# alinjar1996/manipulator_mujoco

Hardware: AMD Instinct MI355X
Metric: candidate rollouts/sec (N×H steps) UR5e scene, 1/2/4/8 MI355X (higher is better)
Workload: dtype f32; 1 GPU; C3 scene_mjx: UR5e+Hand-E arm + object.xml box (URD/scene_mjx.xml), Newton(1 it, 5 ls), 4096 candidates x 50 steps per GPU, order-10 Bernstein, dt 0.05; candidates_per_gpu=4096, horizon=50, global_batch=4096, parallelism=dp1 (candidate shards; key exchange), world_size_seen=1, backend=single process, gpus_visible=1, launcher=single process, exchange=none (one rank: the fused atomic-min key is the global best)

## Files before the change

### manipulator_mujoco_amd/csrc/dev_model.h

```cpp
#pragma once
#include <algorithm>
#include <atomic>
#include <cfloat>
#include <cmath>
#include <cstdarg>
#include <cstdio>
#include <cstring>
#include <limits>
#include <string>
#include <thread>
#include <vector>

#include "../../include/mpcr.h"
#include "model_frames.h"
#include "rollout.h"

namespace mpcr {

struct DevOptions {
  int newton_reuse = 1;
  int m_slab = 0;
  int w2_lead_max = W2_LEAD_MAX;
  uint64_t start_scramble = 0;
};
// ... 314 lines not shown
  }
  {
    int ts[DX_NTREE], te[DX_NTREE];
    bool ok = true;
    for (int t = 0; t < DX_NTREE; t++) ts[t] = te[t] = -1;
    for (int i = 0; i < m.nv && ok; i++) {
      const int b = d.dof_body[i], t = b >= 0 ? d.body_tree[b] : -1;
      if (t < 0 || t >= DX_NTREE) { ok = false; break; }
      if (ts[t] < 0) ts[t] = i;
      else if (te[t] != i) ok = false;
      te[t] = i + 1;
    }
    for (int i = 0; i < m.nv && ok; i++) {
      const int t = d.body_tree[d.dof_body[i]];
      d.mc_c0[i] = std::min(ts[t] & ~3, SmemW::NVW - SmemW::MCW);
      if (te[t] - d.mc_c0[i] > SmemW::MCW) ok = false;
    }
    d.mc_n = ok && m.nv * SmemW::MCW <= SmemW::MC ? m.nv : 0;
    if (opt.m_slab) d.mc_n = 0;
    d.w2_lead_max = std::max(-1, std::min(W2_LEAD_MAX, opt.w2_lead_max));
  }
  for (int i = 0; i < m.nq; i++) d.qpos_init[i] = (float)m.qpos_init[i];
  for (int i = 0; i < m.nv; i++) d.qvel_init[i] = (float)m.qvel_init[i];
  std::vector<int> gmap(m.ngeom, -1);
  int ng = 0;
  for (int p = 0; p < m.npair; p++)
    for (int g : {m.pair_geom1[p], m.pair_geom2[p]})
      if (gmap[g] < 0) gmap[g] = ng++;
  if (ng > DX_NG || ng > WAVE) return dev_fail(err, MPCR_EMODEL, "%d collision geoms > %d", ng, DX_NG < WAVE ? DX_NG : WAVE);
  d.ngeom = ng;
  for (int g = 0; g < m.ngeom; g++) {
    int i = gmap[g];
    if (i < 0) continue;
    int b = m.geom_bodyid[g];
    d.geom_type[i] = m.geom_type[g];
    d.geom_rbound[i] = (float)m.geom_rbound[g];
    d.geom_hulladr[i] = m.geom_hulladr[g];
    d.geom_hullnum[i] = m.geom_hullnum[g];
    d.geom_lutadr[i] = lutadr[g];
    d.geom_faceadr[i] = m.geom_faceadr[g];
    d.geom_facenum[i] = m.geom_faceadr[g] >= 0 ? m.geom_facenum[g] : 0;
    d.geom_cornadr[i] = m.geom_cornadr[g];
    for (int k = 0; k < 3; k++) d.geom_size[i][k] = (float)m.geom_size[g][k];
    if (dmap[b] >= 0) {
      d.geom_body[i] = dmap[b];
      for (int k = 0; k < 3; k++) d.geom_pos[i][k] = (float)m.geom_pos[g][k];
      for (int k = 0; k < 4; k++) d.geom_quat[i][k] = (float)m.geom_quat[g][k];
    } else {
      d.geom_body[i] = -1;
      double r[3], q[4];
      step_detail::rot(r, f.wquat[b], m.geom_pos[g]);
// ... 254 lines not shown
```

### manipulator_mujoco_amd/csrc/engine.hip

```cpp
#include <hip/hip_runtime.h>
#include <dlfcn.h>

#include <algorithm>
#include <atomic>
#include <cmath>
#include <cstdarg>
#include <cstdio>
#include <cstring>
#include <string>
#include <vector>

#include "../../include/mpcr.h"
#include "mpcr_device.h"

#include "rollout.h"
#include "dev_model.h"
#include "step_table.h"

#ifndef MPCR_SEG_STEPS_DEFAULT
#define MPCR_SEG_STEPS_DEFAULT 7
#endif
#ifndef MPCR_SEG_GROUPS_DEFAULT
#define MPCR_SEG_GROUPS_DEFAULT 2
#endif
// ... 289 lines not shown
  HIPCHK(hipSetDevice(device));
  hipDeviceProp_t prop;
  HIPCHK(hipGetDeviceProperties(&prop, device));
  if (std::strncmp(prop.gcnArchName, "gfx950", 6) != 0)
    return fail(MPCR_ENODEV, "device %d is %s; libmpcr is built for gfx950 only", device, prop.gcnArchName);
  auto* e = new mpcr_engine;
  auto refuse = [e](int rc) { mpcr_engine_free(e); return rc; };
  e->device = device;
  e->max_n = max_n;
  e->H = horizon;
  e->nbasis = nbasis;
  e->host = m->m;
  const mpcr_model_t& h = e->host;
  DevOptions opt;
  opt.newton_reuse = env_int_or("MPCR_NEWTON_REUSE", 1);
  opt.m_slab = env_int_or("MPCR_M_SLAB", 0);
  opt.w2_lead_max = env_int_or("MPCR_W2_LEAD_MAX", W2_LEAD_MAX);
  opt.start_scramble = g_start_scramble.load();
  DevTables t;
  std::string err;
  if (int rc = compile_dev_model(h, opt, e->dev, t, err)) return refuse(fail(rc, "%s", err.c_str()));
  e->wide = needs_wide(h, e->dev);
  std::vector<StepTable> step;
  if (!e->wide) {
    step.resize(1);
    if (build_step_table(h, step[0]) != 0) return refuse(fail(MPCR_EMODEL, "model exceeds the step table's capacities"));
  }
  DevBufs& mem = e->mem;
  if (h.nhullv > 0) {
    e->dev.hull_vert = as_gmem(mem.upload(t.hull_vert));
    e->dev.hull_info = as_gmem(mem.upload(t.hull_info));
    e->dev.hull_adjv = as_gmem(mem.upload(t.hull_adjv));
    e->dev.hull_head = as_gmem(mem.upload(t.hull_head));
    e->dev.hull_lut = as_gmem(mem.upload(t.hull_lut));
  }
  if (h.nface > 0) {
    e->dev.face_plane = as_gmem(mem.upload(t.face_plane));
    e->dev.face_vinfo = as_gmem(mem.upload(t.face_vinfo));
    e->dev.face_vert = as_gmem(mem.alloc<int>(h.nfacev, h.face_vert, h.nfacev));
    e->dev.vert_finfo = as_gmem(mem.upload(t.vert_finfo));
    e->dev.vert_face = as_gmem(mem.alloc<int>(h.nvface, h.vert_face, h.nvface));
    e->dev.cone_cell = as_gmem(mem.upload(t.cone_cell));
    e->dev.cone_face = as_gmem(mem.upload(t.cone_face));
  }
  static_assert(sizeof(DevModel) % alignof(mpcr::StepTable) == 0, "the step table's alignment behind the device model");
  const int nc = h.nctrl;
  const size_t rows = (size_t)max_n + 1;
  const size_t nhints = 2 * (size_t)max_n * (e->wide ? SmemW::NHINT : 1);
  e->d_model = reinterpret_cast<DevModel*>(mem.alloc<char>(sizeof(DevModel) + sizeof(StepTable),
                                                           reinterpret_cast<const char*>(&e->dev), sizeof(DevModel)));
  if (e->d_model && !e->wide &&
      hipMemcpy(e->d_model + 1, step.data(), sizeof(StepTable), hipMemcpyHostToDevice) != hipSuccess)
    mem.rc = MPCR_EHIP;
  e->d_pdot = mem.alloc<float>((size_t)horizon * nbasis, pdot, (size_t)horizon * nbasis);
  e->d_in = mem.alloc<float>((size_t)max_n * nc * (horizon > nbasis ? horizon : nbasis));
  e->d_cost = mem.alloc<float>((size_t)max_n * 4);
  e->d_theta = mem.alloc<float>((size_t)max_n * nc * horizon);
  e->d_thetadot = mem.alloc<float>((size_t)max_n * nc * horizon);
  e->d_key = mem.alloc<unsigned long long>(1);
  e->d_status = mem.alloc<int>(max_n);
  e->d_idx = mem.alloc<int>(max_n);
  e->d_slot_prev = mem.alloc<float>(rows * (h.nslot > 0 ? h.nslot : 1));
  e->d_jx = mem.alloc<float>(rows * (e->wide ? (SmemW::MAXEFC - SmemW::JL + 1) * SmemW::LDJ
                                             : (SmemN::MAXEFC - SmemN::JL + 1) * SmemN::LDJ));
  e->d_hints = mem.alloc<short>(nhints);
  e->d_pace = mem.alloc<unsigned>(MPCR_PACE_SLOTS);
  e->d_mslab = mem.alloc<float>(rows * (e->wide ? SmemW::NVW * SmemW::LD : 1));
  e->d_td = mem.alloc<float>(rows * (size_t)(nc > 0 ? nc : 1) * (size_t)horizon);
  if (!mem.rc && (hipMemset(e->d_hints, 0xff, sizeof(short) * nhints) != hipSuccess ||
                  hipMemset(e->d_pace, 0xff, sizeof(unsigned) * MPCR_PACE_SLOTS) != hipSuccess))
    mem.rc = MPCR_EHIP;
  if (e->wide) {
    e->seg_steps = env_int_or("MPCR_SEG_STEPS", MPCR_SEG_STEPS_DEFAULT);
    e->seg_groups = std::max(1, std::min(MPCR_SEG_MAXG, env_int_or("MPCR_SEG_GROUPS", MPCR_SEG_GROUPS_DEFAULT)));
    if (e->seg_steps > 0 && e->seg_steps < horizon) {
// ... 834 lines not shown
```

### manipulator_mujoco_amd/csrc/model_frames.h

```cpp
#pragma once
#include <math.h>
#include <stdint.h>
#include <string.h>

#include "../../include/mpcr_model.h"

namespace mpcr {

enum { ST_BK_FREE = 1, ST_BK_HINGE = 2, ST_BK_SLIDE = 3, ST_BK_WELD = 4 };

namespace step_detail {
inline void qmul(double r[4], const double a[4], const double b[4]) {
  const double t[4] = {a[0] * b[0] - a[1] * b[1] - a[2] * b[2] - a[3] * b[3],
                       a[0] * b[1] + a[1] * b[0] + a[2] * b[3] - a[3] * b[2],
                       a[0] * b[2] - a[1] * b[3] + a[2] * b[0] + a[3] * b[1],
                       a[0] * b[3] + a[1] * b[2] - a[2] * b[1] + a[3] * b[0]};
  memcpy(r, t, sizeof(t));
}
inline void q2m(double m[9], const double q[4]) {
  const double w = q[0], x = q[1], y = q[2], z = q[3];
  m[0] = 1 - 2 * (y * y + z * z); m[1] = 2 * (x * y - w * z); m[2] = 2 * (x * z + w * y);
  m[3] = 2 * (x * y + w * z); m[4] = 1 - 2 * (x * x + z * z); m[5] = 2 * (y * z - w * x);
  m[6] = 2 * (x * z - w * y); m[7] = 2 * (y * z + w * x); m[8] = 1 - 2 * (x * x + y * y);
}
// ... 51 lines not shown
      f.anc[i] = -1;
    } else {
      memcpy(f.bpos[i], m.body_pos[b], sizeof(f.bpos[i]));
      memcpy(f.bquat[i], m.body_quat[b], sizeof(f.bquat[i]));
      f.anc[i] = f.dmap[p];
    }
    if (f.kind[i] == ST_BK_FREE) f.anc[i] = -1;
    f.depth[i] = f.anc[i] < 0 ? 1 : f.depth[f.anc[i]] + 1;
    f.maxdepth = f.depth[i] > f.maxdepth ? f.depth[i] : f.maxdepth;
    int t = -1;
    for (int k = 0; k < f.ntree; k++)
      if (roots[k] == m.body_rootid[b]) t = k;
    if (t < 0) { roots[f.ntree] = m.body_rootid[b]; t = f.ntree++; }
    f.tree[i] = t;
  }
  for (int i = 0; i < m.nv; i++) {
    const int j = m.dof_jntid[i], sub = i - m.jnt_dofadr[j];
    f.dof_kind[i] = m.jnt_type[j] == MPCR_JNT_HINGE ? 0 : (m.jnt_type[j] == MPCR_JNT_SLIDE ? 1 : (sub < 3 ? 2 : 3));
    f.dof_sub[i] = sub < 3 ? sub : sub - 3;
  }
  return 0;
}

inline float pair_margin_f(const mpcr_model_t& m, int p) { return (float)(m.pair_margin[p] - m.pair_gap[p]); }
inline bool pair_frictionless(const mpcr_model_t& m, int p) { return m.pair_condim[p] == 1; }
inline bool jnt_limit_row(const mpcr_model_t& m, int j) {
  return m.jnt_limited[j] && (m.jnt_type[j] == MPCR_JNT_SLIDE || m.jnt_type[j] == MPCR_JNT_HINGE);
}
inline float jnt_range_f(const mpcr_model_t& m, int j, int k) { return (float)m.jnt_range[j][k]; }
inline float jnt_margin_f(const mpcr_model_t& m, int j) { return (float)m.jnt_margin[j]; }
inline float dof_invweight_f(const mpcr_model_t& m, int i) { return (float)m.dof_invweight0[i]; }
inline float eq_diag_f(const mpcr_model_t& m, int e) {
  double diag = 0;
  if (m.eq_type[e] == MPCR_EQ_JOINT) {
    diag = m.dof_invweight0[m.jnt_dofadr[m.eq_obj1[e]]];
    if (m.eq_obj2[e] >= 0) diag += m.dof_invweight0[m.jnt_dofadr[m.eq_obj2[e]]];
  } else if (m.eq_type[e] == MPCR_EQ_CONNECT) {
    diag = m.body_invweight0[m.eq_obj1[e]][0] + m.body_invweight0[m.eq_obj2[e]][0];
  }
  return (float)diag;
}

}
```

### manipulator_mujoco_amd/csrc/rollout.hip

```cpp
#pragma once
#include "rollout.h"
#include "step_table.h"
#include "../../include/mpcr_model.h"

namespace mpcr {

#ifdef MPCR_PROFILE
#define PROF_DECL unsigned long long prof_acc[32] = {0}; unsigned long long prof_last = __builtin_amdgcn_s_memtime();
#define STAMP(i)                                              \
  do {                                                        \
    unsigned long long now_ = __builtin_amdgcn_s_memtime();   \
    prof_acc[i] += now_ - prof_last;                          \
    prof_last = now_;                                         \
  } while (0)
#define PROF_FLUSH                                                          \
  if (lane == 0 && args.prof)                                               \
    for (int i_ = 0; i_ < 32; i_++) atomicAdd(&args.prof[i_ + 32 * (threadIdx.x >> 6)], prof_acc[i_]);
#ifdef MPCR_PROFILE_COUNTS
#define PROF_COUNT(m, i)                                                                  \
  do {                                                                                    \
    if ((m)->prof && (int)__lane_id() == __builtin_ctzll(__ballot(1))) atomicAdd((m)->prof + (i), 1ull); \
  } while (0)
#else
#define PROF_COUNT(m, i)
// ... 11 lines not shown
#define PROF_DECL
#define STAMP(i)
#define PROF_FLUSH
#define PROF_COUNT(m, i)
#endif
#define PACE_SETPRIO() \
  if (pace) {   \
  const int ahead = __popcll(__ballot(lane < 16 && lane != pace_own && pace_v != ~0u && pace_v > (unsigned)t)); \
  if (ahead >= 3) __builtin_amdgcn_s_setprio(3); \
  else if (ahead == 2) __builtin_amdgcn_s_setprio(2); \
  else if (ahead == 1) __builtin_amdgcn_s_setprio(1); \
  else __builtin_amdgcn_s_setprio(0); \
  }

#ifndef MPCR_CB_SKIP
#define MPCR_CB_SKIP 1
#endif
#ifdef MPCR_STOP_AFTER
#define STOP_AT(k) \
  if (MPCR_STOP_AFTER == (k)) continue;
#else
#define STOP_AT(k)
#endif


#if defined(__HIP_DEVICE_COMPILE__)
#define ASSUME_GLOBAL(p) __builtin_assume(!__builtin_amdgcn_is_shared((const void*)(p)) && \
                                          !__builtin_amdgcn_is_private((const void*)(p)))
#define ASSUME_LDS(p) __builtin_assume(__builtin_amdgcn_is_shared((const void*)(p)))
#define ASSUME_PRIVATE(p) __builtin_assume(__builtin_amdgcn_is_private((const void*)(p)))
#else
#define ASSUME_GLOBAL(p)
#define ASSUME_LDS(p)
#define ASSUME_PRIVATE(p)
#endif
__device__ __forceinline__ const MPCR_GMEM DevModel* uniform_model(const DevModel* p) {
  const unsigned long long a = reinterpret_cast<unsigned long long>(p);
  const unsigned lo = __builtin_amdgcn_readfirstlane((unsigned)a), hi = __builtin_amdgcn_readfirstlane((unsigned)(a >> 32));
  return reinterpret_cast<const MPCR_GMEM DevModel*>(((unsigned long long)hi << 32) | lo);
}

#ifndef MPCR_STEP_TABLE
#define MPCR_STEP_TABLE 7
#endif
template <class S> constexpr bool kStepKin = !S::WIDE && (MPCR_STEP_TABLE & 1) != 0;
template <class S> constexpr bool kStepDof = !S::WIDE && (MPCR_STEP_TABLE & 2) != 0;
template <class S> constexpr bool kStepRow = !S::WIDE && (MPCR_STEP_TABLE & 4) != 0;
__device__ __forceinline__ const StepTable* step_table(const DevModel* m) {
  return reinterpret_cast<const StepTable*>(m + 1);
}
template <class R>
__device__ __forceinline__ float4 recq(const R& r, int q) {
  return reinterpret_cast<const float4*>(&r)[q];
}

__device__ __forceinline__ float rdlane(float v, int l) {
  return __int_as_float(__builtin_amdgcn_readlane(__float_as_int(v), l));
}
template <int CTRL>
__device__ __forceinline__ float dppf(float v) {
  return __int_as_float(__builtin_amdgcn_update_dpp(0, __float_as_int(v), CTRL, 0xF, 0xF, false));
}
template <int CTRL, int ROWS>
__device__ __forceinline__ float dppf_rows(float v) {
  return __int_as_float(__builtin_amdgcn_update_dpp(0, __float_as_int(v), CTRL, ROWS, 0xF, false));
}
__device__ __forceinline__ float wsum_ref(float v) {
  v += dppf<0xB1>(v);
  v += dppf<0x4E>(v);
  v += dppf<0x124>(v);
  v += dppf<0x128>(v);
  v += dppf_rows<0x142, 0xA>(v);
// ... 1303 lines not shown
    idx[0] = ia; idx[1] = ib; idx[2] = ic; idx[3] = beats(bap, bbp) ? iap : ibp;
  }
#pragma unroll
  for (int j = 0; j < 4; j++) {
    bool dup = idx[j] < 0;
#pragma unroll
    for (int t = 0; t < j; t++) dup |= idx[t] == idx[j];
    const int L = idx[j] < 0 ? 0 : idx[j];
    const float Pj[3] = {__shfl(P[0], L), __shfl(P[1], L), __shfl(P[2], L)};
    const float dj = __shfl(dk, L);
    if (lane == q) {
      dist[j] = dup ? 1e30f : dj;
#pragma unroll
      for (int e = 0; e < 3; e++) { pos[j][e] = Pj[e] - 0.5f * dj * nr[e] + c[e]; nrm[j][e] = sg * nr[e]; }
    }
  }
  if (lane == q) nsl = 4;
  PSTAMP(m, 28);
}

template <class S>
__device__ __forceinline__ int narrow_lane(const DevModel* __restrict__ m, const S& s, short* hints, int p, float dist[4],
                            float pos[4][3], float nrm[4][3], float* dbg = nullptr) {
  const int g1 = m->pair_g1[p], g2 = m->pair_g2[p];
  const int func = m->pair_func[p];
  const float* x1 = s.gxpos[g1];
  const float* x2 = s.gxpos[g2];
  const float* R1 = s.gxmat[g1];
  const float* R2 = s.gxmat[g2];
  const float* s1 = m->geom_size[g1];
  const float* s2 = m->geom_size[g2];
#pragma unroll
  for (int k = 0; k < 4; k++) dist[k] = 1e30f;
  if (func == 0) {
    float n[3] = {R1[2], R1[5], R1[8]}, ax[3] = {R2[2], R2[5], R2[8]};
    float r = s2[0], hl = s2[1];
#pragma unroll
    for (int k = 0; k < 2; k++) {
      float sg = k == 0 ? 1.f : -1.f, e[3], dif[3];
#pragma unroll
      for (int c = 0; c < 3; c++) { e[c] = x2[c] + sg * hl * ax[c]; dif[c] = e[c] - x1[c]; }
      float d = dot3(n, dif) - r;
      dist[k] = d;
#pragma unroll
      for (int c = 0; c < 3; c++) { pos[k][c] = e[c] - n[c] * (r + 0.5f * d); nrm[k][c] = n[c]; }
    }
    return 2;
  }
  if (func == 1) {
    const float n[3] = {R1[2], R1[5], R1[8]};
    float w[3];
#pragma unroll
    for (int k = 0; k < 3; k++) w[k] = s2[k] * (n[0] * R2[k] + n[1] * R2[3 + k] + n[2] * R2[6 + k]);
    const int c0 = (w[0] < 0.f ? 1 : 0) | (w[1] < 0.f ? 2 : 0) | (w[2] < 0.f ? 4 : 0);
// ... 551 lines not shown
  for (int c = 0; c < 4; c++) {
    if (c < nsl && dist[c] < mg) {
      if (o < S::MAXACT) {
        float f[9];
        make_frame(f, nrm[c]);
        s.con_pos[o][0] = pos[c][0]; s.con_pos[o][1] = pos[c][1]; s.con_pos[o][2] = pos[c][2];
#pragma unroll
        for (int e = 0; e < S::FRAMEW; e++) s.con_frame[o][e] = f[e];
        s.con_dist[o] = dist[c];
        s.con_pair[o] = p;
      }
      o++;
    }
  }
}

template <class S>
__device__ __forceinline__ void emit_contacts(const DevModel* __restrict__ m, S& s, const RolloutArgs& args, int b,
                                              int t, int H, bool valid, int p, int nsl, const float dist[4],
                                              const float pos[4][3], const float nrm[4][3], float& cost_c,
                                              SlotHist<S>& sh, int k) {
  int act = 0;
  if (valid) {
    const int sa = m->pair_slotadr[p];
    if (sa >= 0) {
      const int ns = m->pair_ncon[p];
#pragma unroll
      for (int c = 0; c < 4; c++) {
        if (c < ns) {
          const float d = dist[c];
          if (d < 0.f) cost_c += 1.f;
          if (SlotHist<S>::NC > 0 && k < SlotHist<S>::NC) {
            float prev = 0.f;
#pragma unroll
            for (int j = 0; j < SlotHist<S>::NC; j++) prev = j == k ? sh.v[j][c] : prev;
            if (t > 0) cost_c += fmaxf(prev * (1.f - 0.005f) - d, 0.f);
#pragma unroll
            for (int j = 0; j < SlotHist<S>::NC; j++) sh.v[j][c] = j == k ? d : sh.v[j][c];
          } else {
            float* cp = args.slot_prev + (size_t)b * m->nslot;
            if (t > 0) cost_c += fmaxf(cp[sa + c] * (1.f - 0.005f) - d, 0.f);
            cp[sa + c] = d;
          }
          if (args.trace_slots && b < args.n) args.trace_slots[((size_t)b * H + t) * m->nslot + sa + c] = d;
        }
      }
    }
    if (!(m->disableflags & 16)) {
      const float mg = m->pair_margin[p];
#pragma unroll
      for (int c = 0; c < 4; c++) act += (c < nsl && dist[c] < mg) ? 1 : 0;
    }
  }
  int tot;
  const int pre = wscan_excl(act, tot);
  const int base = s.ncon;
  if (act) put_contacts(m, s, base + pre, p, nsl, dist, pos, nrm);
  sync();
  if ((threadIdx.x & (WAVE - 1)) == 0) s.ncon = base + tot;
  sync();
}


template <class T>
struct LsPtT { T alpha, cost, d0, d1; bool full; };
template <class S>
using LsReal = typename std::conditional<S::WIDE, double, float>::type;

__device__ __forceinline__ bool ell_row(int src) { return (src >> 24) == 5; }
__device__ __forceinline__ bool ell_head(int src) { return (src >> 24) == 5 && (src & 15) == 0; }
__device__ __forceinline__ int ell_pair(int src) { return (src >> 4) & 1023; }

// ... 1001 lines not shown
        float wr[3];
        cross(wr, cv, rr);
#pragma unroll
        for (int k = 0; k < 3; k++) { F[k] += vl * (cv[3 + k] + wr[k]); Tv[k] = va * cv[k]; }
      }
      cross(tq, rr, F);
      tq[0] += Tv[0]; tq[1] += Tv[1]; tq[2] += Tv[2];
      s.cfrc[lane][0] = f[0] + vf[0] - tq[0];
      s.cfrc[lane][1] = f[1] + vf[1] - tq[1];
      s.cfrc[lane][2] = f[2] + vf[2] - tq[2];
      s.cfrc[lane][3] = f[3] + vf[3] - F[0];
      s.cfrc[lane][4] = f[4] + vf[4] - F[1];
      s.cfrc[lane][5] = f[5] + vf[5] - F[2];
    }
    sync();
    STAMP(4);
    STOP_AT(4)
    if constexpr (MFMA_DYN) {
      const int mr = lane & 15, kq = lane >> 4;
      const mfx4 z4 = {0.f, 0.f, 0.f, 0.f};
      const mfx4 P = mm16<2>([&](int i, int c) { return (i < nv && c < 6) ? s.fvec[i][c] : 0.f; },
                             [&](int c, int j) { return (j < nv && c < 6) ? s.cdof[j][c] : 0.f; }, z4, lane);
      const int j = mr;
#pragma unroll
      for (int v = 0; v < 4; v++) {
        const int i = 4 * kq + v;
        if (i < nv && j < nv) {
          if ((m->dof_chainmask[i] >> j) & 1u) {
            const float x = i == j ? P[v] + m->dof_armature[i] : P[v];
            m_set(i, j, x);
            m_set(j, i, x);
          } else if (!((m->dof_chainmask[j] >> i) & 1u)) {
            m_set(i, j, 0.f);
          }
        } else {
          m_set(i, j, i == j ? 1.f : 0.f);
        }
      }
      const uint32_t sub = mr < nv ? m->dof_submask[mr] : 0u;
      const mfx4 fb = mm16<4>([&](int, int b) { return ((sub >> b) & 1u) ? 1.f : 0.f; },
                              [&](int b, int c) { return (b < nb && c < 6) ? s.cfrc[b][c] : 0.f; }, z4, lane);
#pragma unroll
      for (int v = 0; v < 4; v++)
        if (mr < 6) dscr[(4 * kq + v) * 8 + mr] = fb[v];
      sync();
    } else {
    for (int idx = lane; idx < NVW * NVW; idx += WAVE) {
      const int i = idx >> S::LOG_NVW, j = idx & (NVW - 1);
      float v = 0.f;
      if (i < nv && j < nv) {
        if ((m->dof_chainmask[i] >> j) & 1u) {
#pragma unroll
          for (int k = 0; k < 6; k++) v = fmaf(s.cdof[j][k], s.fvec[i][k], v);
        } else if ((m->dof_chainmask[j] >> i) & 1u) {
#pragma unroll
          for (int k = 0; k < 6; k++) v = fmaf(s.cdof[i][k], s.fvec[j][k], v);
        }
        if (i == j) v += m->dof_armature[i];
      } else if (i == j) {
        v = 1.f;
// ... 64 lines not shown
    if (run_coll) {
      if (pass == 0) { do_list = true; do_narrow = !swapm; }
      else do_narrow = swapm && s.ncvx > m->w2_lead_max;
    } else if (pass == 1) {
      bool posted = true;
      if constexpr (S::SPLIT) {
        int guard = 0;
        while (__hip_atomic_load(&s.ctok_[0], __ATOMIC_ACQUIRE, __HIP_MEMORY_SCOPE_WORKGROUP) != t + 1 &&
               ++guard < (1 << 22))
          __builtin_amdgcn_s_sleep(1);
        if (guard >= (1 << 22)) { status |= 1 << 10; posted = false; }
      }
      do_narrow = posted && s.ncvx <= m->w2_lead_max;
    }
    if (do_list || do_narrow) {
    if (do_list) {
      if (lane == 0) { s.ncon = 0; s.ncvx = 0; }
      sync();
    }
    const int k_lo = do_narrow ? 0 : m->cvx_base / WAVE, p_hi = do_list ? m->npair : min(m->npair, m->cvx_base);
    for (int k = k_lo; k * WAVE < p_hi; k++) {
      const int p = lane + k * WAVE;
      const bool valid = p < m->npair;
      const int func = valid ? m->pair_func[p] : -1;
      const bool defer = S::WIDE && func >= 9;
      bool run = valid && (defer ? do_list : do_narrow);
      if (run && m->pair_slotadr[p] < 0) {
        const int g1 = m->pair_g1[p], g2 = m->pair_g2[p];
        const float dx = s.gxpos[g2][0] - s.gxpos[g1][0], dy = s.gxpos[g2][1] - s.gxpos[g1][1],
                    dz = s.gxpos[g2][2] - s.gxpos[g1][2];
        if (m->geom_type[g1] != 0) {
          run = sqrtf(dx * dx + dy * dy + dz * dz) <= m->geom_rbound[g1] + m->geom_rbound[g2] + m->pair_margin[p];
          if constexpr (S::WIDE) {
            if (run && func == 9 && (m->geom_type[g1] == 6 || m->geom_type[g2] == 6)) {
              const bool b1 = m->geom_type[g1] == 6;
              const int gb = b1 ? g1 : g2;
              const float sg = b1 ? 1.f : -1.f;
              float d[3] = {sg * dx, sg * dy, sg * dz}, l[3];
              mtv(l, s.gxmat[gb], d);
              float o2 = 0.f;
#pragma unroll
              for (int k2 = 0; k2 < 3; k2++) {
                const float e = fmaxf(fabsf(l[k2]) - m->geom_size[gb][k2], 0.f);
                o2 += e * e;
              }
              run = sqrtf(o2) <= m->geom_rbound[b1 ? g2 : g1] + m->pair_margin[p];
            }
          }
        } else {
// ... 223 lines not shown
      } else
      if (lane < m->njnt && !(m->disableflags & 32) && m->jnt_limited[lane] &&
          (m->jnt_type[lane] == 2 || m->jnt_type[lane] == 3)) {
        const float q = s.qpos[m->jnt_qposadr[lane]];
        if (q - m->jnt_range[lane][0] < m->jnt_margin[lane]) { nlim_l++; lsides |= 1; }
        if (m->jnt_range[lane][1] - q < m->jnt_margin[lane]) { nlim_l++; lsides |= 2; }
      }
      int nlim;
      const int lim_pre = wscan_excl(nlim_l, nlim);
      int ntr = 0, tsides = 0;
      if constexpr (S::WIDE) {
        if (!(m->disableflags & 32))
          for (int t = 0; t < m->nten; t++) {
            if (!m->ten_limited[t]) continue;
            const float dx = s.tenp[t][1][0] - s.tenp[t][0][0], dy = s.tenp[t][1][1] - s.tenp[t][0][1],
                        dz = s.tenp[t][1][2] - s.tenp[t][0][2];
            const float len = sqrtf(dx * dx + dy * dy + dz * dz);
            if (len - m->ten_range[t][0] < m->ten_margin[t]) { tsides |= 1 << (2 * t); ntr++; }
            if (m->ten_range[t][1] - len < m->ten_margin[t]) { tsides |= 2 << (2 * t); ntr++; }
          }
      }
      const bool ell = S::WIDE && m->cone == 1;
      int ncr = 0;
      if (lane < ncon) ncr = m->pair_condim[s.con_pair[lane]] == 1 ? 1 : (ell ? 3 : 4);
      int ncrow;
      const int con_pre = wscan_excl(ncr, ncrow);
      int nefc = neq + nlim + ntr + ncrow;
      int keep_con = ncon;
      if (nefc > S::MAXEFC) {
        const int room = S::MAXEFC - neq - nlim - ntr;
        const unsigned long long fit = __ballot(lane < ncon && con_pre + ncr <= room);
        keep_con = __popcll(fit);
        nefc = neq + nlim + ntr + (keep_con > 0 ? wshfl(con_pre + ncr, keep_con - 1) : 0);
        status |= 1;
      }
      if (lane < neq)
        s.efc_src[lane] = S::WIDE ? ((1 << 24) | (m->eqrow_eq[lane] << 4) | m->eqrow_k[lane]) : ((1 << 24) | (lane << 4));
      if (nlim_l) {
        int o = neq + lim_pre;
        if (lsides & 1) s.efc_src[o++] = (2 << 24) | (lane << 4) | 0;
        if (lsides & 2) s.efc_src[o++] = (2 << 24) | (lane << 4) | 1;
      }
      if constexpr (S::WIDE) {
        if (lane == 0 && ntr) {
          int o = neq + nlim;
          for (int t = 0; t < m->nten; t++)
            for (int side = 0; side < 2; side++)
              if ((tsides >> (2 * t + side)) & 1) s.efc_src[o++] = (4 << 24) | (t << 4) | side;
        }
      }
      if (lane < keep_con) {
        const int o = neq + nlim + ntr + con_pre;
        s.con_row[lane] = o;
        if (ncr == 3) {
          const int p = s.con_pair[lane];
          for (int r = 0; r < 3; r++) s.efc_src[o + r] = (5 << 24) | (lane << 14) | (p << 4) | r;
        } else {
          for (int r = 0; r < ncr; r++) s.efc_src[o + r] = (3 << 24) | (lane << 4) | r;
        }
      }
      {
        bool cross = false;
        if (lane < keep_con) {
          const int4 ji = m->pair_jinfo[s.con_pair[lane]];
          cross = ji.x != 0 && ji.y != 0 && ji.z != ji.w;
        }
        coupled = m->eq_cross || __ballot(cross) != 0ull;
      }
      if (lane == 0) s.nefc = nefc;
      sync();
      const int nsimple = neq + nlim + ntr;
      for (int idx = lane + rl0; idx < nsimple * NVW; idx += rls) {
        const int r = idx >> S::LOG_NVW, i = idx & (NVW - 1);
        const int src = s.efc_src[r], kind = src >> 24, id = (src >> 4) & 0xfffff, side = src & 15;
        float v = 0.f;
        if (S::WIDE && kind == 1 && side > 0) {
          const int comp = side - 1;
          if (i < nv) {
            const float* cd = s.cdof[i];
#pragma unroll
            for (int e2 = 0; e2 < 2; e2++) {
              const int bb = e2 == 0 ? m->eq_b1[id] : m->eq_b2[id];
              if (bb >= 0 && ((m->body_dofmask[bb] >> i) & 1u)) {
                const int tr = m->body_tree[bb];
                float r[3] = {s.eqp[id][e2][0] - s.com[tr][0], s.eqp[id][e2][1] - s.com[tr][1],
                              s.eqp[id][e2][2] - s.com[tr][2]}, cr[3];
                cross(cr, cd, r);
                const float jv = cd[3 + comp] + cr[comp];
                v += e2 == 0 ? jv : -jv;
              }
            }
          }
        } else if (kind == 1) {
          const int j1 = m->eq_j1[id], j2 = m->eq_j2[id];
// ... 8 lines not shown
            const float dif[3] = {s.tenp[id][1][0] - s.tenp[id][0][0], s.tenp[id][1][1] - s.tenp[id][0][1],
                                  s.tenp[id][1][2] - s.tenp[id][0][2]};
            const float il = 1.f / fmaxf(sqrtf(dot3(dif, dif)), kMinVal);
            const float* cd = s.cdof[i];
#pragma unroll
            for (int e2 = 0; e2 < 2; e2++) {
              const int bb = m->ten_body[id][e2];
              if (bb >= 0 && ((m->body_dofmask[bb] >> i) & 1u)) {
                const int tr = m->body_tree[bb];
                float rr[3] = {s.tenp[id][e2][0] - s.com[tr][0], s.tenp[id][e2][1] - s.com[tr][1],
                               s.tenp[id][e2][2] - s.com[tr][2]}, cr[3];
                cross(cr, cd, rr);
                const float jp = (dif[0] * (cd[3] + cr[0]) + dif[1] * (cd[4] + cr[1]) + dif[2] * (cd[5] + cr[2])) * il;
                v += e2 == 0 ? -jp : jp;
              }
            }
            if (side) v = -v;
          }
        } else if (i == m->jnt_dofadr[id]) {
          v = side == 0 ? 1.f : -1.f;
        }
        jstore(s, gx, r, i, v);
      }
      for (int idx = lane + rl0; idx < keep_con * NVW; idx += rls) {
        const int c = idx >> S::LOG_NVW, i = idx & (NVW - 1);
        const int p = s.con_pair[c];
        const int4 ji = m->pair_jinfo[p];
        float jd[3] = {0.f, 0.f, 0.f};
        if (i < nv) {
          const float* cd = s.cdof[i];
#pragma unroll
          for (int side = 0; side < 2; side++) {
            if (((unsigned)(side == 0 ? ji.x : ji.y) >> i) & 1u) {
              const int tr = side == 0 ? ji.z : ji.w;
              float r[3] = {s.con_pos[c][0] - s.com[tr][0], s.con_pos[c][1] - s.com[tr][1],
                            s.con_pos[c][2] - s.com[tr][2]}, cr[3];
              cross(cr, cd, r);
              const float sg = side == 0 ? -1.f : 1.f;
              jd[0] += sg * (cd[3] + cr[0]); jd[1] += sg * (cd[4] + cr[1]); jd[2] += sg * (cd[5] + cr[2]);
            }
          }
        }
        float fw[9];
        const float* f = s.con_frame[c];
        if constexpr (S::FRAMEW == 3) {
          make_frame(fw, s.con_frame[c]);
          f = fw;
        }
        const float jn = f[0] * jd[0] + f[1] * jd[1] + f[2] * jd[2];
        const int off = s.con_row[c];
        if (m->pair_condim[p] == 1) {
          jstore(s, gx, off, i, jn);
        } else if (S::WIDE && m->cone == 1) {
          jstore(s, gx, off + 0, i, jn);
          jstore(s, gx, off + 1, i, f[3] * jd[0] + f[4] * jd[1] + f[5] * jd[2]);
          jstore(s, gx, off + 2, i, f[6] * jd[0] + f[7] * jd[1] + f[8] * jd[2]);
        } else {
          const float mu = m->pair_friction[p];
          const float jt1 = f[3] * jd[0] + f[4] * jd[1] + f[5] * jd[2];
          const float jt2 = f[6] * jd[0] + f[7] * jd[1] + f[8] * jd[2];
          jstore(s, gx, off + 0, i, jn + mu * jt1);
          jstore(s, gx, off + 1, i, jn - mu * jt1);
          jstore(s, gx, off + 2, i, jn + mu * jt2);
          jstore(s, gx, off + 3, i, jn - mu * jt2);
        }
      }
      if (rows_j) block_sync();
      else sync();
      if constexpr (kStepRow<S>) {
        for (int r = lane + rl0; r < nefc; r += rls) {
          const int src = s.efc_src[r], kind = src >> 24, id = (src >> 4) & 0xfffff, side = src & 15;
          const StepTable* st = step_table(m);
          float pos;
          int ri;
          if (kind == 1) {
            const int j1 = m->eq_j1[id], j2 = m->eq_j2[id];
            const float* c = m->eq_data[id];
            const float q1 = s.qpos[m->jnt_qposadr[j1]] - m->jnt_qpos0[j1];
            if (j2 >= 0) {
              const float dif = s.qpos[m->jnt_qposadr[j2]] - m->jnt_qpos0[j2];
              pos = q1 - (c[0] + dif * (c[1] + dif * (c[2] + dif * (c[3] + dif * c[4]))));
            } else {
              pos = q1 - c[0];
            }
            ri = ST_ROW_EQ + id;
          } else if (kind == 2) {
            ri = ST_ROW_JNT + id;
            const float4 j3 = recq(st->row[ri], 3);
            const float q = s.qpos[__float_as_int(j3.z)];
            pos = side == 0 ? q - j3.x : j3.y - q;
          } else {
            ri = ST_ROW_PAIR + s.con_pair[id];
            pos = s.con_dist[id];
          }
          const float4 a0 = recq(st->row[ri], 0), a1 = recq(st->row[ri], 1), a2 = recq(st->row[ri], 2);
          const float vel = jdot(s, gx, r, s.qvel);
          const float dpos = pos - a2.x;
          const float x = fabsf(dpos * a0.z);
          float imp;
          if (x >= 1.f) {
            imp = a0.y;
          } else if (x <= 0.f) {
            imp = a0.x;
          } else {
            const int fl = __float_as_int(a2.z);
            const float mid = a0.w, power = a2.w;
            float y;
            if (fl & ST_POW1) y = x;
            else if (fl & ST_POW2) y = x <= mid ? x * x * a1.x : 1.f - (1.f - x) * (1.f - x) * a1.y;
            else if (x <= mid) y = powf(x, power) / powf(mid, power - 1.f);
            else y = 1.f - powf(1.f - x, power) / powf(1.f - mid, power - 1.f);
            imp = a0.x + y * (a0.y - a0.x);
          }
          const float R = fmaxf((1.f - imp) / imp * a2.y, kMinVal);
          s.efc_D[r] = 1.f / R;
          s.efc_aref[r] = -a1.w * vel - a1.z * imp * dpos;
          if (args.dbg && b == 0 && t == H - 1 && r < DBG_MAXROW) {
            float* o = args.dbg + DBG_ROW + 3 * r;
// ... 599 lines not shown
```

### manipulator_mujoco_amd/csrc/step_table.h

```cpp
#pragma once
#include <math.h>
#include <stdint.h>
#include <string.h>

#include "model_frames.h"

namespace mpcr {

constexpr int ST_NB = 32, ST_NV = 32, ST_NP = 768, ST_NJ = 32, ST_NEQ = 8;
constexpr int ST_ROW_PAIR = 0, ST_ROW_JNT = ST_NP, ST_ROW_EQ = ST_NP + ST_NJ, ST_NROW = ST_NP + ST_NJ + ST_NEQ;
constexpr float ST_MINVAL = 1e-15f, ST_MINIMP = 0.0001f, ST_MAXIMP = 0.9999f;

enum { ST_ANCHOR0 = 1 };
enum {
  ST_POW2 = 1,
  ST_POW1 = 2,
  ST_LIMITED = 4,
  ST_CONDIM1 = 8
};
struct alignas(16) StepBody {
  int32_t kind, anc, qposadr;
  float qpos0;
  float bquat[4];
  float bpos[3], pad0;
  float axis[3], pad1;
  float ipos[3], pad2;
  float jpos[3], pad3;
  float R[3][4];
};
struct alignas(16) StepDof {
  int32_t body, kind, tree, sub;
  float axis[3], pad0;
  float jpos[3], pad1;
};
struct alignas(16) StepRow {
  float dmin, dmax, iwidth, mid;
  float imid, i1mid, K, B;
  float margin, diag;
  int32_t flags;
  float power;
  float range[2];
  int32_t qposadr, dofadr;
};

struct alignas(16) StepTable {
  int32_t flags, nbody, pad[2];
  StepBody body[ST_NB];
  StepDof dof[ST_NV];
  StepRow row[ST_NROW];
};

namespace step_detail {
inline double clampd(double x, double lo, double hi) { return x < lo ? lo : (x > hi ? hi : x); }

inline void row_params(StepRow& r, const double solref[2], const double solimp[5], double timestep, int disableflags) {
  double dmin = clampd(solimp[0], (double)ST_MINIMP, (double)ST_MAXIMP);
  double dmax = clampd(solimp[1], (double)ST_MINIMP, (double)ST_MAXIMP);
  double width = solimp[2], mid = solimp[3];
  const double power = solimp[4];
  const bool flat = (float)dmin == (float)dmax || (float)width <= ST_MINVAL;
  double iwidth = 1.0 / width, imid = 1.0 / mid, i1mid = 1.0 / (1.0 - mid);
  if (flat) {
    dmin = dmax = 0.5 * ((double)(float)dmin + (double)(float)dmax);
    iwidth = 0.0; mid = 0.5; imid = 2.0; i1mid = 2.0;
  }
  const double d = clampd(solimp[1], (double)ST_MINIMP, (double)ST_MAXIMP);
  double tc = solref[0];
  const double dr = solref[1];
  double K, B;
  if ((float)tc > 0.f) {
    if (!(disableflags & MPCR_DSBL_REFSAFE) && tc < 2.0 * timestep) tc = 2.0 * timestep;
    K = 1.0 / (d * d * tc * tc * dr * dr);
// ... 41 lines not shown
        if (r.jpos[k] != 0.f) anchor0 = false;
      }
    }
  }
  t.flags = anchor0 ? ST_ANCHOR0 : 0;
  for (int i = 0; i < m.nv; i++) {
    StepDof& r = t.dof[i];
    const int j = m.dof_jntid[i];
    r.body = f.dmap[m.dof_bodyid[i]];
    r.kind = f.dof_kind[i];
    r.tree = r.body >= 0 ? f.tree[r.body] : -1;
    r.sub = f.dof_sub[i];
    for (int k = 0; k < 3; k++) { r.axis[k] = (float)m.jnt_axis[j][k]; r.jpos[k] = (float)m.jnt_pos[j][k]; }
  }
  for (int p = 0; p < m.npair; p++) {
    StepRow& r = t.row[ST_ROW_PAIR + p];
    row_params(r, m.pair_solref[p], m.pair_solimp[p], m.timestep, m.disableflags);
    const double mu = m.pair_friction[p];
    const double invw = m.body_invweight0[m.geom_bodyid[m.pair_geom1[p]]][0] +
                        m.body_invweight0[m.geom_bodyid[m.pair_geom2[p]]][0];
    r.margin = pair_margin_f(m, p);
    r.diag = (float)(pair_frictionless(m, p) ? invw : invw * (1.0 + mu * mu));
    if (pair_frictionless(m, p)) r.flags |= ST_CONDIM1;
    r.qposadr = r.dofadr = -1;
  }
  for (int j = 0; j < m.njnt; j++) {
    StepRow& r = t.row[ST_ROW_JNT + j];
    row_params(r, m.jnt_solref[j], m.jnt_solimp[j], m.timestep, m.disableflags);
    r.margin = jnt_margin_f(m, j);
    r.diag = dof_invweight_f(m, m.jnt_dofadr[j]);
    if (jnt_limit_row(m, j)) r.flags |= ST_LIMITED;
    r.range[0] = jnt_range_f(m, j, 0);
    r.range[1] = jnt_range_f(m, j, 1);
    r.qposadr = m.jnt_qposadr[j];
    r.dofadr = m.jnt_dofadr[j];
  }
  for (int e = 0; e < m.neq; e++) {
    StepRow& r = t.row[ST_ROW_EQ + e];
    row_params(r, m.eq_solref[e], m.eq_solimp[e], m.timestep, m.disableflags);
    r.margin = 0.f;
    r.diag = eq_diag_f(m, e);
    r.qposadr = r.dofadr = -1;
  }
  return 0;
}

}
```

Baseline: 2.744 million rollouts/s.

## Pack per-pair and equality setup into 16-byte load records for step kernel

```diff
diff --git a/manipulator_mujoco_amd/csrc/dev_model.h b/manipulator_mujoco_amd/csrc/dev_model.h
--- a/manipulator_mujoco_amd/csrc/dev_model.h
+++ b/manipulator_mujoco_amd/csrc/dev_model.h
@@ -360,11 +360,8 @@
   }
   for (int i = 0; i < m.nq; i++) d.qpos_init[i] = (float)m.qpos_init[i];
   for (int i = 0; i < m.nv; i++) d.qvel_init[i] = (float)m.qvel_init[i];
-  std::vector<int> gmap(m.ngeom, -1);
-  int ng = 0;
-  for (int p = 0; p < m.npair; p++)
-    for (int g : {m.pair_geom1[p], m.pair_geom2[p]})
-      if (gmap[g] < 0) gmap[g] = ng++;
+  int gmap[MPCR_MAX_GEOM];
+  const int ng = pair_geom_map(m, gmap);
   if (ng > DX_NG || ng > WAVE) return dev_fail(err, MPCR_EMODEL, "%d collision geoms > %d", ng, DX_NG < WAVE ? DX_NG : WAVE);
   d.ngeom = ng;
   for (int g = 0; g < m.ngeom; g++) {
diff --git a/manipulator_mujoco_amd/csrc/engine.hip b/manipulator_mujoco_amd/csrc/engine.hip
--- a/manipulator_mujoco_amd/csrc/engine.hip
+++ b/manipulator_mujoco_amd/csrc/engine.hip
@@ -335,9 +335,12 @@
   if (int rc = compile_dev_model(h, opt, e->dev, t, err)) return refuse(fail(rc, "%s", err.c_str()));
   e->wide = needs_wide(h, e->dev);
   std::vector<StepTable> step;
+  std::vector<StepRecords> recs;
   if (!e->wide) {
     step.resize(1);
-    if (build_step_table(h, step[0]) != 0) return refuse(fail(MPCR_EMODEL, "model exceeds the step table's capacities"));
+    recs.resize(1);
+    if (build_step_table(h, step[0]) != 0 || build_step_records(h, recs[0]) != 0)
+      return refuse(fail(MPCR_EMODEL, "model exceeds the step table's capacities"));
   }
   DevBufs& mem = e->mem;
   if (h.nhullv > 0) {
@@ -360,10 +363,13 @@
   const int nc = h.nctrl;
   const size_t rows = (size_t)max_n + 1;
   const size_t nhints = 2 * (size_t)max_n * (e->wide ? SmemW::NHINT : 1);
-  e->d_model = reinterpret_cast<DevModel*>(mem.alloc<char>(sizeof(DevModel) + sizeof(StepTable),
+  static_assert(sizeof(StepTable) % alignof(mpcr::StepRecords) == 0, "the load records' alignment behind the step table");
+  e->d_model = reinterpret_cast<DevModel*>(mem.alloc<char>(sizeof(DevModel) + sizeof(StepTable) + sizeof(StepRecords),
                                                            reinterpret_cast<const char*>(&e->dev), sizeof(DevModel)));
   if (e->d_model && !e->wide &&
-      hipMemcpy(e->d_model + 1, step.data(), sizeof(StepTable), hipMemcpyHostToDevice) != hipSuccess)
+      (hipMemcpy(e->d_model + 1, step.data(), sizeof(StepTable), hipMemcpyHostToDevice) != hipSuccess ||
+       hipMemcpy(reinterpret_cast<char*>(e->d_model + 1) + sizeof(StepTable), recs.data(), sizeof(StepRecords),
+                 hipMemcpyHostToDevice) != hipSuccess))
     mem.rc = MPCR_EHIP;
   e->d_pdot = mem.alloc<float>((size_t)horizon * nbasis, pdot, (size_t)horizon * nbasis);
   e->d_in = mem.alloc<float>((size_t)max_n * nc * (horizon > nbasis ? horizon : nbasis));
diff --git a/manipulator_mujoco_amd/csrc/model_frames.h b/manipulator_mujoco_amd/csrc/model_frames.h
--- a/manipulator_mujoco_amd/csrc/model_frames.h
+++ b/manipulator_mujoco_amd/csrc/model_frames.h
@@ -97,6 +97,15 @@
   return 0;
 }
 
+inline int pair_geom_map(const mpcr_model_t& m, int gmap[MPCR_MAX_GEOM]) {
+  for (int g = 0; g < MPCR_MAX_GEOM; g++) gmap[g] = -1;
+  int ng = 0;
+  for (int p = 0; p < m.npair; p++)
+    for (int g : {m.pair_geom1[p], m.pair_geom2[p]})
+      if (gmap[g] < 0) gmap[g] = ng++;
+  return ng;
+}
+
 inline float pair_margin_f(const mpcr_model_t& m, int p) { return (float)(m.pair_margin[p] - m.pair_gap[p]); }
 inline bool pair_frictionless(const mpcr_model_t& m, int p) { return m.pair_condim[p] == 1; }
 inline bool jnt_limit_row(const mpcr_model_t& m, int j) {
diff --git a/manipulator_mujoco_amd/csrc/rollout.hip b/manipulator_mujoco_amd/csrc/rollout.hip
--- a/manipulator_mujoco_amd/csrc/rollout.hip
+++ b/manipulator_mujoco_amd/csrc/rollout.hip
@@ -57,6 +57,11 @@
 #else
 #define STOP_AT(k)
 #endif
+#if defined(MPCR_PROFILE) && defined(MPCR_PROFILE_ROWS)
+#define ROWS_STAMP(i) STAMP(i)
+#else
+#define ROWS_STAMP(i)
+#endif
 
 
 #if defined(__HIP_DEVICE_COMPILE__)
@@ -76,13 +81,17 @@
 }
 
 #ifndef MPCR_STEP_TABLE
-#define MPCR_STEP_TABLE 7
+#define MPCR_STEP_TABLE 15
 #endif
 template <class S> constexpr bool kStepKin = !S::WIDE && (MPCR_STEP_TABLE & 1) != 0;
 template <class S> constexpr bool kStepDof = !S::WIDE && (MPCR_STEP_TABLE & 2) != 0;
 template <class S> constexpr bool kStepRow = !S::WIDE && (MPCR_STEP_TABLE & 4) != 0;
+template <class S> constexpr bool kStepLoad = !S::WIDE && (MPCR_STEP_TABLE & 8) != 0;
 __device__ __forceinline__ const StepTable* step_table(const DevModel* m) {
   return reinterpret_cast<const StepTable*>(m + 1);
+}
+__device__ __forceinline__ const StepRecords* step_records(const DevModel* m) {
+  return reinterpret_cast<const StepRecords*>(step_table(m) + 1);
 }
 template <class R>
 __device__ __forceinline__ float4 recq(const R& r, int q) {
@@ -1432,14 +1441,23 @@
 template <class S>
 __device__ __forceinline__ int narrow_lane(const DevModel* __restrict__ m, const S& s, short* hints, int p, float dist[4],
                             float pos[4][3], float nrm[4][3], float* dbg = nullptr) {
-  const int g1 = m->pair_g1[p], g2 = m->pair_g2[p];
-  const int func = m->pair_func[p];
+  [[maybe_unused]] float4 q0 = {0.f, 0.f, 0.f, 0.f};
+  [[maybe_unused]] float sz1[3], sz2[3];
+  if constexpr (kStepLoad<S>) {
+    const StepPairSetup& ps = step_records(m)->pair[p];
+    q0 = recq(ps, 0);
+    const float4 q2 = recq(ps, 2), q3 = recq(ps, 3);
+    sz1[0] = q2.x; sz1[1] = q2.y; sz1[2] = q2.z;
+    sz2[0] = q3.x; sz2[1] = q3.y; sz2[2] = q3.z;
+  }
+  const int g1 = kStepLoad<S> ? __float_as_int(q0.z) : m->pair_g1[p], g2 = kStepLoad<S> ? __float_as_int(q0.w) : m->pair_g2[p];
+  const int func = kStepLoad<S> ? __float_as_int(q0.x) : m->pair_func[p];
   const float* x1 = s.gxpos[g1];
   const float* x2 = s.gxpos[g2];
   const float* R1 = s.gxmat[g1];
   const float* R2 = s.gxmat[g2];
-  const float* s1 = m->geom_size[g1];
-  const float* s2 = m->geom_size[g2];
+  const float* s1 = kStepLoad<S> ? sz1 : m->geom_size[g1];
+  const float* s2 = kStepLoad<S> ? sz2 : m->geom_size[g2];
 #pragma unroll
   for (int k = 0; k < 4; k++) dist[k] = 1e30f;
   if (func == 0) {
@@ -2037,9 +2055,15 @@
                                               SlotHist<S>& sh, int k) {
   int act = 0;
   if (valid) {
-    const int sa = m->pair_slotadr[p];
+    float4 q0 = {0.f, 0.f, 0.f, 0.f}, q1 = q0;
+    if constexpr (kStepLoad<S>) {
+      const StepPairSetup& ps = step_records(m)->pair[p];
+      q0 = recq(ps, 0);
+      q1 = recq(ps, 1);
+    }
+    const int sa = kStepLoad<S> ? __float_as_int(q0.y) : m->pair_slotadr[p];
     if (sa >= 0) {
-      const int ns = m->pair_ncon[p];
+      const int ns = kStepLoad<S> ? __float_as_int(q1.x) >> 16 : m->pair_ncon[p];
 #pragma unroll
       for (int c = 0; c < 4; c++) {
         if (c < ns) {
@@ -2062,7 +2086,7 @@
       }
     }
     if (!(m->disableflags & 16)) {
-      const float mg = m->pair_margin[p];
+      const float mg = kStepLoad<S> ? q1.w : m->pair_margin[p];
 #pragma unroll
       for (int c = 0; c < 4; c++) act += (c < nsl && dist[c] < mg) ? 1 : 0;
     }
@@ -3110,6 +3134,28 @@
       const mfx4 P = mm16<2>([&](int i, int c) { return (i < nv && c < 6) ? s.fvec[i][c] : 0.f; },
                              [&](int c, int j) { return (j < nv && c < 6) ? s.cdof[j][c] : 0.f; }, z4, lane);
       const int j = mr;
+      if constexpr (kStepLoad<S>) {
+        uint32_t cmi[4];
+#pragma unroll
+        for (int v = 0; v < 4; v++) cmi[v] = m->dof_chainmask[4 * kq + v];
+        const uint32_t cmj = m->dof_chainmask[j];
+        const float arm = m->dof_armature[j];
+#pragma unroll
+        for (int v = 0; v < 4; v++) {
+          const int i = 4 * kq + v;
+          if (i < nv && j < nv) {
+            if ((cmi[v] >> j) & 1u) {
+              const float x = i == j ? P[v] + arm : P[v];
+              m_set(i, j, x);
+              m_set(j, i, x);
+            } else if (!((cmj >> i) & 1u)) {
+              m_set(i, j, 0.f);
+            }
+          } else {
+            m_set(i, j, i == j ? 1.f : 0.f);
+          }
+        }
+      } else {
 #pragma unroll
       for (int v = 0; v < 4; v++) {
         const int i = 4 * kq + v;
@@ -3124,6 +3170,7 @@
         } else {
           m_set(i, j, i == j ? 1.f : 0.f);
         }
+      }
       }
       const uint32_t sub = mr < nv ? m->dof_submask[mr] : 0u;
       const mfx4 fb = mm16<4>([&](int, int b) { return ((sub >> b) & 1u) ? 1.f : 0.f; },
@@ -3234,9 +3281,30 @@
     for (int k = k_lo; k * WAVE < p_hi; k++) {
       const int p = lane + k * WAVE;
       const bool valid = p < m->npair;
-      const int func = valid ? m->pair_func[p] : -1;
+      float4 ps0 = {0.f, 0.f, 0.f, 0.f}, ps1 = ps0;
+      if constexpr (kStepLoad<S>) {
+        if (valid) {
+          const StepPairSetup& ps = step_records(m)->pair[p];
+          ps0 = recq(ps, 0);
+          ps1 = recq(ps, 1);
+        }
+      }
+      const int func = valid ? (kStepLoad<S> ? __float_as_int(ps0.x) : m->pair_func[p]) : -1;
       const bool defer = S::WIDE && func >= 9;
       bool run = valid && (defer ? do_list : do_narrow);
+      if constexpr (kStepLoad<S>) {
+        if (run && __float_as_int(ps0.y) < 0) {
+          const int g1 = __float_as_int(ps0.z), g2 = __float_as_int(ps0.w);
+          const float dx = s.gxpos[g2][0] - s.gxpos[g1][0], dy = s.gxpos[g2][1] - s.gxpos[g1][1],
+                      dz = s.gxpos[g2][2] - s.gxpos[g1][2];
+          if ((__float_as_int(ps1.x) & 255) != 0) {
+            run = sqrtf(dx * dx + dy * dy + dz * dz) <= ps1.y + ps1.z + ps1.w;
+          } else {
+            const float* R1 = s.gxmat[g1];
+            run = R1[2] * dx + R1[5] * dy + R1[8] * dz <= ps1.z + ps1.w;
+          }
+        }
+      } else
       if (run && m->pair_slotadr[p] < 0) {
         const int g1 = m->pair_g1[p], g2 = m->pair_g2[p];
         const float dx = s.gxpos[g2][0] - s.gxpos[g1][0], dy = s.gxpos[g2][1] - s.gxpos[g1][1],
@@ -3506,6 +3574,13 @@
       }
       const bool ell = S::WIDE && m->cone == 1;
       int ncr = 0;
+      float4 pj = {0.f, 0.f, 0.f, 0.f};
+      if constexpr (kStepLoad<S>) {
+        if (lane < ncon) {
+          pj = recq(step_table(m)->row[ST_ROW_PAIR + s.con_pair[lane]], 3);
+          ncr = (__float_as_int(pj.z) >> 16) & 1 ? 1 : 4;
+        }
+      } else
       if (lane < ncon) ncr = m->pair_condim[s.con_pair[lane]] == 1 ? 1 : (ell ? 3 : 4);
       int ncrow;
       const int con_pre = wscan_excl(ncr, ncrow);
@@ -3545,6 +3620,11 @@
       }
       {
         bool cross = false;
+        if constexpr (kStepLoad<S>) {
+          const int tr = __float_as_int(pj.z);
+          cross = lane < keep_con && __float_as_int(pj.x) != 0 && __float_as_int(pj.y) != 0 &&
+                  (tr & 255) != ((tr >> 8) & 255);
+        } else
         if (lane < keep_con) {
           const int4 ji = m->pair_jinfo[s.con_pair[lane]];
           cross = ji.x != 0 && ji.y != 0 && ji.z != ji.w;
@@ -3553,7 +3633,29 @@
       }
       if (lane == 0) s.nefc = nefc;
       sync();
+      ROWS_STAMP(23);
       const int nsimple = neq + nlim + ntr;
+      if constexpr (kStepLoad<S>) {
+        static_assert((ST_NEQ & (ST_NEQ - 1)) == 0 && (ST_NJ & (ST_NJ - 1)) == 0, "the masks below need powers of two");
+        for (int idx = lane + rl0; idx < nsimple * NVW; idx += rls) {
+          const int r = idx >> S::LOG_NVW, i = idx & (NVW - 1);
+          const int src = s.efc_src[r], kind = src >> 24, id = (src >> 4) & 0xfffff, side = src & 15;
+          const StepEq& eq = step_records(m)->eq[id & (ST_NEQ - 1)];
+          const float4 e0 = recq(eq, 0), e1 = recq(eq, 1), e2 = recq(eq, 2);
+          const int ldof = step_table(m)->row[ST_ROW_JNT + (id & (ST_NJ - 1))].dofadr;
+          float v = 0.f;
+          if (kind == 1) {
+            if (i == __float_as_int(e0.y)) v += 1.f;
+            if (__float_as_int(e0.z) >= 0 && i == __float_as_int(e0.w)) {
+              const float dif = s.qpos[__float_as_int(e0.z)] - e1.y;
+              v -= e1.w + dif * (2.f * e2.x + dif * (3.f * e2.y + dif * 4.f * e2.z));
+            }
+          } else if (i == ldof) {
+            v = side == 0 ? 1.f : -1.f;
+          }
+          jstore(s, gx, r, i, v);
+        }
+      } else
       for (int idx = lane + rl0; idx < nsimple * NVW; idx += rls) {
         const int r = idx >> S::LOG_NVW, i = idx & (NVW - 1);
         const int src = s.efc_src[r], kind = src >> 24, id = (src >> 4) & 0xfffff, side = src & 15;
@@ -3608,10 +3710,22 @@
         }
         jstore(s, gx, r, i, v);
       }
+      ROWS_STAMP(24);
       for (int idx = lane + rl0; idx < keep_con * NVW; idx += rls) {
         const int c = idx >> S::LOG_NVW, i = idx & (NVW - 1);
         const int p = s.con_pair[c];
-        const int4 ji = m->pair_jinfo[p];
+        int4 ji;
+        float muq = 0.f;
+        bool condim1 = false;
+        if constexpr (kStepLoad<S>) {
+          const float4 q3 = recq(step_table(m)->row[ST_ROW_PAIR + p], 3);
+          const int tr = __float_as_int(q3.z);
+          ji = make_int4(__float_as_int(q3.x), __float_as_int(q3.y), tr & 255, (tr >> 8) & 255);
+          condim1 = (tr >> 16) & 1;
+          muq = q3.w;
+        } else {
+          ji = m->pair_jinfo[p];
+        }
         float jd[3] = {0.f, 0.f, 0.f};
         if (i < nv) {
           const float* cd = s.cdof[i];
@@ -3635,14 +3749,14 @@
         }
         const float jn = f[0] * jd[0] + f[1] * jd[1] + f[2] * jd[2];
         const int off = s.con_row[c];
-        if (m->pair_condim[p] == 1) {
+        if (kStepLoad<S> ? condim1 : m->pair_condim[p] == 1) {
           jstore(s, gx, off, i, jn);
         } else if (S::WIDE && m->cone == 1) {
           jstore(s, gx, off + 0, i, jn);
           jstore(s, gx, off + 1, i, f[3] * jd[0] + f[4] * jd[1] + f[5] * jd[2]);
           jstore(s, gx, off + 2, i, f[6] * jd[0] + f[7] * jd[1] + f[8] * jd[2]);
         } else {
-          const float mu = m->pair_friction[p];
+          const float mu = kStepLoad<S> ? muq : m->pair_friction[p];
           const float jt1 = f[3] * jd[0] + f[4] * jd[1] + f[5] * jd[2];
           const float jt2 = f[6] * jd[0] + f[7] * jd[1] + f[8] * jd[2];
           jstore(s, gx, off + 0, i, jn + mu * jt1);
@@ -3653,12 +3767,35 @@
       }
       if (rows_j) block_sync();
       else sync();
+      ROWS_STAMP(25);
       if constexpr (kStepRow<S>) {
         for (int r = lane + rl0; r < nefc; r += rls) {
           const int src = s.efc_src[r], kind = src >> 24, id = (src >> 4) & 0xfffff, side = src & 15;
           const StepTable* st = step_table(m);
           float pos;
           int ri;
+          float4 a0, a1, a2;
+          if constexpr (kStepLoad<S>) {
+            ri = kind == 1 ? ST_ROW_EQ + id : (kind == 2 ? ST_ROW_JNT + id : ST_ROW_PAIR + s.con_pair[kind == 3 ? id : 0]);
+            a0 = recq(st->row[ri], 0); a1 = recq(st->row[ri], 1); a2 = recq(st->row[ri], 2);
+            const float4 j3 = recq(st->row[ri], 3);
+            if (kind == 1) {
+              const StepEq& eq = step_records(m)->eq[id & (ST_NEQ - 1)];
+              const float4 e0 = recq(eq, 0), e1 = recq(eq, 1), e2 = recq(eq, 2);
+              const float q1 = s.qpos[__float_as_int(e0.x)] - e1.x;
+              if (__float_as_int(e0.z) >= 0) {
+                const float dif = s.qpos[__float_as_int(e0.z)] - e1.y;
+                pos = q1 - (e1.z + dif * (e1.w + dif * (e2.x + dif * (e2.y + dif * e2.z))));
+              } else {
+                pos = q1 - e1.z;
+              }
+            } else if (kind == 2) {
+              const float q = s.qpos[__float_as_int(j3.z)];
+              pos = side == 0 ? q - j3.x : j3.y - q;
+            } else {
+              pos = s.con_dist[id];
+            }
+          } else {
           if (kind == 1) {
             const int j1 = m->eq_j1[id], j2 = m->eq_j2[id];
             const float* c = m->eq_data[id];
@@ -3679,7 +3816,8 @@
             ri = ST_ROW_PAIR + s.con_pair[id];
             pos = s.con_dist[id];
           }
-          const float4 a0 = recq(st->row[ri], 0), a1 = recq(st->row[ri], 1), a2 = recq(st->row[ri], 2);
+          a0 = recq(st->row[ri], 0); a1 = recq(st->row[ri], 1); a2 = recq(st->row[ri], 2);
+          }
           const float vel = jdot(s, gx, r, s.qvel);
           const float dpos = pos - a2.x;
           const float x = fabsf(dpos * a0.z);
diff --git a/manipulator_mujoco_amd/csrc/step_table.h b/manipulator_mujoco_amd/csrc/step_table.h
--- a/manipulator_mujoco_amd/csrc/step_table.h
+++ b/manipulator_mujoco_amd/csrc/step_table.h
@@ -1,5 +1,6 @@
 #pragma once
 #include <math.h>
+#include <stddef.h>
 #include <stdint.h>
 #include <string.h>
 
@@ -43,11 +44,34 @@
   int32_t qposadr, dofadr;
 };
 
+struct alignas(16) StepPairJ {
+  uint32_t mask1, mask2;
+  int32_t trees;
+  float mu;
+};
+
 struct alignas(16) StepTable {
   int32_t flags, nbody, pad[2];
   StepBody body[ST_NB];
   StepDof dof[ST_NV];
   StepRow row[ST_NROW];
+};
+
+struct alignas(16) StepPairSetup {
+  int32_t func, slotadr, g1, g2;
+  int32_t types;
+  float rbound1, rbound2, margin;
+  float size1[3], pad0;
+  float size2[3], pad1;
+};
+struct alignas(16) StepEq {
+  int32_t qadr1, dadr1, qadr2, dadr2;
+  float qpos0_1, qpos0_2, c0, c1;
+  float c2, c3, c4, pad;
+};
+struct alignas(16) StepRecords {
+  StepPairSetup pair[ST_NP];
+  StepEq eq[ST_NEQ];
 };
 
 namespace step_detail {
@@ -135,7 +159,14 @@
     r.margin = pair_margin_f(m, p);
     r.diag = (float)(pair_frictionless(m, p) ? invw : invw * (1.0 + mu * mu));
     if (pair_frictionless(m, p)) r.flags |= ST_CONDIM1;
-    r.qposadr = r.dofadr = -1;
+    StepPairJ q;
+    const int b1 = f.dmap[m.geom_bodyid[m.pair_geom1[p]]], b2 = f.dmap[m.geom_bodyid[m.pair_geom2[p]]];
+    q.mask1 = b1 >= 0 ? m.body_dofmask[f.id[b1]] : 0u;
+    q.mask2 = b2 >= 0 ? m.body_dofmask[f.id[b2]] : 0u;
+    q.trees = (b1 >= 0 ? f.tree[b1] : 0) | (b2 >= 0 ? f.tree[b2] : 0) << 8 | (pair_frictionless(m, p) ? 1 << 16 : 0);
+    q.mu = (float)m.pair_friction[p];
+    static_assert(sizeof(q) == 16 && offsetof(StepRow, range) == 48 && sizeof(StepRow) == 64, "quad 3");
+    memcpy(reinterpret_cast<char*>(&r) + 48, &q, sizeof(q));
   }
   for (int j = 0; j < m.njnt; j++) {
     StepRow& r = t.row[ST_ROW_JNT + j];
@@ -158,4 +189,42 @@
   return 0;
 }
 
-}
+inline int build_step_records(const mpcr_model_t& m, StepRecords& r) {
+  memset(&r, 0, sizeof(r));
+  if (m.npair > ST_NP || m.neq > ST_NEQ || m.njnt > ST_NJ || m.ngeom > MPCR_MAX_GEOM) return -1;
+  int gmap[MPCR_MAX_GEOM];
+  pair_geom_map(m, gmap);
+  for (int p = 0; p < m.npair; p++) {
+    StepPairSetup& s = r.pair[p];
+    const int g1 = m.pair_geom1[p], g2 = m.pair_geom2[p];
+    s.func = m.pair_func[p];
+    s.slotadr = m.pair_slotadr[p];
+    s.g1 = gmap[g1];
+    s.g2 = gmap[g2];
+    s.types = (m.geom_type[g1] & 255) | (m.geom_type[g2] & 255) << 8 | m.pair_ncon[p] << 16;
+    s.rbound1 = (float)m.geom_rbound[g1];
+    s.rbound2 = (float)m.geom_rbound[g2];
+    s.margin = pair_margin_f(m, p);
+    for (int k = 0; k < 3; k++) { s.size1[k] = (float)m.geom_size[g1][k]; s.size2[k] = (float)m.geom_size[g2][k]; }
+  }
+  for (int e = 0; e < m.neq; e++) {
+    StepEq& q = r.eq[e];
+    q.qadr1 = q.dadr1 = q.qadr2 = q.dadr2 = -1;
+    if (m.eq_type[e] != MPCR_EQ_JOINT) continue;
+    const int j1 = m.eq_obj1[e], j2 = m.eq_obj2[e];
+    if (j1 < 0 || j1 >= m.njnt || j2 >= m.njnt) return -1;
+    q.qadr1 = m.jnt_qposadr[j1];
+    q.dadr1 = m.jnt_dofadr[j1];
+    q.qpos0_1 = (float)m.qpos0[m.jnt_qposadr[j1]];
+    if (j2 >= 0) {
+      q.qadr2 = m.jnt_qposadr[j2];
+      q.dadr2 = m.jnt_dofadr[j2];
+      q.qpos0_2 = (float)m.qpos0[m.jnt_qposadr[j2]];
+    }
+    q.c0 = (float)m.eq_data[e][0]; q.c1 = (float)m.eq_data[e][1]; q.c2 = (float)m.eq_data[e][2];
+    q.c3 = (float)m.eq_data[e][3]; q.c4 = (float)m.eq_data[e][4];
+  }
+  return 0;
+}
+
+}
```

After: 2.772 million rollouts/s, median of 6. 1.0% higher.
